# Patryk27/strolle

Hardware: NVIDIA H100
Metric: Mrays/s (+ frames/s) at 1080p-per-GPU Cornell, ReSTIR DI+GI + SVGF; H100 vs CPU restatement of the reference (higher is better)
Workload: dtype f32

## Files before the change

include/strolle_b200.h:

```cpp
#ifndef STROLLE_B200_H
#define STROLLE_B200_H

#include <stddef.h>
#include <stdint.h>

#ifdef __cplusplus
extern "C" {
#endif

typedef struct st_engine st_engine;
typedef uint64_t st_handle;
typedef int32_t st_camera_handle;

enum { ST_OK = 0, ST_ERR_CUDA = -1, ST_ERR_INVALID = -2, ST_ERR_NOT_FOUND = -3, ST_ERR_LIMIT = -4 };

typedef struct st_mesh_triangle {
    float positions[3][3];
    float normals[3][3];
    float uvs[3][2];
    float tangents[3][4];
} st_mesh_triangle;

typedef struct st_material {
    float base_color[4];
// ... 46 lines not shown
typedef struct st_material_textures { st_handle base_color, emissive, metallic_roughness, normal_map; uint32_t mask; } st_material_textures;
int st_set_material_textures(st_engine* e, st_handle material, const st_material_textures* textures);
int st_insert_instance(st_engine* e, st_handle instance, st_handle mesh, st_handle material, const float affine[12]);
int st_remove_instance(st_engine* e, st_handle instance);
int st_insert_light(st_engine* e, st_handle light, const st_light* l);
int st_remove_light(st_engine* e, st_handle light);
int st_update_sun(st_engine* e, float azimuth, float altitude);

int st_create_camera(st_engine* e, const st_camera* camera, st_camera_handle* out);
int st_update_camera(st_engine* e, st_camera_handle camera, const st_camera* desc);
int st_delete_camera(st_engine* e, st_camera_handle camera);

int st_tick(st_engine* e);

int st_render_camera(st_engine* e, st_camera_handle camera, void* host_out, int format);
int st_copy_output(st_engine* e, st_camera_handle camera, void* host_out, int format);
int st_synchronize(st_engine* e);

int st_set_seed_base(st_engine* e, uint32_t base);
int st_set_blue_noise(st_engine* e, const uint8_t* rgba8_256x256);
int st_read_buffer(st_engine* e, st_camera_handle camera, const char* name, float* dst, size_t cap_floats, size_t* count);
int st_read_scene(st_engine* e, const char* name, float* dst, size_t cap_floats, size_t* count);
int st_bvh_depth(st_engine* e, int* depth);
uint32_t st_frame(st_engine* e);
int st_set_frame(st_engine* e, uint32_t frame);
int st_trace_closest(st_engine* e, const float* rays, size_t n, float* out, float* device_ms);
int st_trace_any(st_engine* e, const float* rays, size_t n, uint32_t* out, float* device_ms);
int st_device_math(st_engine* e, int op, const float* a, const float* b, float* out, size_t n);
#define ST_PASS_COUNT 27
int st_enable_timing(st_engine* e, int enabled);
int st_pass_times(st_engine* e, float* ms, uint32_t* launches, int reset);
const char* st_pass_name(int pass);
int st_wavelet_times(st_engine* e, float* ms5, uint32_t* launches5, int reset);
enum { ST_OPT_SVGF_FAST_MATH = 1, ST_OPT_ASYNC_OUTPUT = 2, ST_OPT_HALO_NCCL = 3, ST_OPT_WAVELET_TILED = 4, ST_OPT_WAVELET_TILE_CFG = 5, ST_OPT_FUSE_REPROJECT = 6, ST_OPT_BVH_REUSE = 7, ST_OPT_VARIANCE_TILED = 8, ST_OPT_SHADING_FAST_MATH = 9, ST_OPT_STRIP_FUSED = 10, ST_OPT_FUSED_PASSES = 11, ST_OPT_STRIP_DMA = 12, ST_OPT_WAVELET_PAIRED = 13 };
#define ST_WAVELET_PAIRED_DEFAULT 1
#define ST_STRIP_DMA_DEFAULT (-1)
#define ST_FUSED_PASSES_DEFAULT 1
#define ST_SHADING_FAST_DEFAULT 1
#define ST_VARIANCE_TILED_DEFAULT 1
#define ST_WAVELET_TILED_DEFAULT 15
#define ST_WAVELET_CFG_DEFAULT 0x01000
#define ST_FUSE_REPROJECT_DEFAULT 1
int st_set_option(st_engine* e, int option, int value);
enum { ST_STAT_WAVELET_TILED_LAUNCHES = 1, ST_STAT_WAVELET_TILED_ERRORS = 2, ST_STAT_BVH_GRAFTED_SUBTREES = 3, ST_STAT_VARIANCE_TILED_LAUNCHES = 4,
       ST_STAT_STRIP_PULLED_ROWS = 5 , ST_STAT_LAST_FRAME_FUSED_STRIPS = 6 ,
       ST_STAT_STRIP_FIRST_TIMEOUT = 7  };
int st_get_stat(st_engine* e, int stat, uint64_t* value);
typedef struct st_bvh_builder st_bvh_builder;
int st_bvh_builder_create(st_bvh_builder** out);
void st_bvh_builder_destroy(st_bvh_builder* b);
int st_bvh_builder_build(st_bvh_builder* b, const float* prims11, size_t n, int reuse, float* out, size_t cap_floats, size_t* n_floats,
                         uint32_t* grafted_subtrees, int* depth);
int st_bvh_builder_read(st_bvh_builder* b, float* out, size_t cap_floats);
int st_set_stream(st_engine* e, void* cuda_stream, int external);
int st_count_rays(st_engine* e, int enabled);
int st_ray_count(st_engine* e, uint64_t* rays, int reset);
int st_nccl_unique_id(uint8_t* out128);
int st_nccl_init(st_engine* e, const uint8_t* id128, int rank, int world);
int st_plan_frame(const int* schedule, int n, uint32_t frame, int temporal_reach, char* out, size_t cap);
int st_render_strips(st_engine* e, st_camera_handle camera, void* host_out, int format, int temporal_reach, int gather);
int st_plan_strip_order(const int* schedule, int n, int dma, char* out, size_t cap);
int st_strip_bounds(int height, int world, int* rows_out);
int st_halo_bytes(st_engine* e, uint64_t* bytes);
#define ST_PEER_HANDLE_BYTES 192
int st_peer_export(st_engine* e, st_camera_handle camera, uint8_t* out192);
int st_peer_import(st_engine* e, st_camera_handle camera, const uint8_t* all_handles, int rank, int world);
int st_peer_errors(st_engine* e, st_camera_handle camera, uint32_t* count);
// ... 45 lines not shown
```

rust/strolle-b200-sys/src/lib.rs:

```rust
#![allow(non_camel_case_types, clippy::too_many_arguments)]

use std::os::raw::{c_char, c_int, c_void};

#[repr(C)] pub struct st_engine { _private: [u8; 0] }
#[repr(C)] pub struct st_multi { _private: [u8; 0] }
#[repr(C)] pub struct st_bvh_builder { _private: [u8; 0] }
pub type st_handle = u64;
pub type st_camera_handle = i32;

pub const ST_OK: c_int = 0;
pub const ST_ERR_CUDA: c_int = -1;
pub const ST_ERR_INVALID: c_int = -2;
pub const ST_ERR_NOT_FOUND: c_int = -3;
pub const ST_ERR_LIMIT: c_int = -4;

#[repr(C)] #[derive(Clone, Copy, Debug, Default)]
pub struct st_mesh_triangle { pub positions: [[f32; 3]; 3], pub normals: [[f32; 3]; 3], pub uvs: [[f32; 2]; 3], pub tangents: [[f32; 4]; 3] }
#[repr(C)] #[derive(Clone, Copy, Debug, Default)]
pub struct st_material { pub base_color: [f32; 4], pub emissive: [f32; 4], pub perceptual_roughness: f32, pub metallic: f32, pub reflectance: f32, pub ior: f32, pub alpha_blend: i32 }
#[repr(C)] #[derive(Clone, Copy, Debug, Default)]
pub struct st_material_textures { pub base_color: st_handle, pub emissive: st_handle, pub metallic_roughness: st_handle, pub normal_map: st_handle, pub mask: u32 }
pub const ST_LIGHT_POINT: i32 = 1;
pub const ST_LIGHT_SPOT: i32 = 2;
#[repr(C)] #[derive(Clone, Copy, Debug, Default)]
pub struct st_light { pub kind: i32, pub position: [f32; 3], pub radius: f32, pub color: [f32; 3], pub range: f32, pub direction: [f32; 3], pub angle: f32 }
pub const ST_MODE_IMAGE: i32 = 0;
pub const ST_MODE_DI_DIFFUSE: i32 = 1;
pub const ST_MODE_DI_SPECULAR: i32 = 2;
pub const ST_MODE_GI_DIFFUSE: i32 = 3;
pub const ST_MODE_GI_SPECULAR: i32 = 4;
pub const ST_MODE_BVH_HEATMAP: i32 = 5;
pub const ST_MODE_REFERENCE: i32 = 6;
#[repr(C)] #[derive(Clone, Copy, Debug)]
pub struct st_camera { pub mode: i32, pub denoise: i32, pub ref_depth: i32, pub width: u32, pub height: u32, pub transform: [f32; 16], pub projection: [f32; 16] }
pub const ST_FORMAT_RGBA32F: c_int = 0;
pub const ST_FORMAT_RGBA8_SRGB: c_int = 1;
pub const ST_PASS_COUNT: usize = 27;
pub const ST_PEER_HANDLE_BYTES: usize = 192;

pub const ST_OPT_SVGF_FAST_MATH: c_int = 1;
pub const ST_OPT_ASYNC_OUTPUT: c_int = 2;
pub const ST_OPT_HALO_NCCL: c_int = 3;
pub const ST_OPT_WAVELET_TILED: c_int = 4;
pub const ST_OPT_WAVELET_TILE_CFG: c_int = 5;
pub const ST_OPT_FUSE_REPROJECT: c_int = 6;
pub const ST_OPT_BVH_REUSE: c_int = 7;
pub const ST_OPT_VARIANCE_TILED: c_int = 8;
pub const ST_OPT_SHADING_FAST_MATH: c_int = 9;
pub const ST_OPT_STRIP_FUSED: c_int = 10;
pub const ST_OPT_FUSED_PASSES: c_int = 11;
pub const ST_OPT_STRIP_DMA: c_int = 12;
pub const ST_OPT_WAVELET_PAIRED: c_int = 13;
pub const ST_STAT_WAVELET_TILED_LAUNCHES: c_int = 1;
pub const ST_STAT_WAVELET_TILED_ERRORS: c_int = 2;
pub const ST_STAT_BVH_GRAFTED_SUBTREES: c_int = 3;
pub const ST_STAT_VARIANCE_TILED_LAUNCHES: c_int = 4;
pub const ST_STAT_STRIP_PULLED_ROWS: c_int = 5;
pub const ST_STAT_LAST_FRAME_FUSED_STRIPS: c_int = 6;
pub const ST_STAT_STRIP_FIRST_TIMEOUT: c_int = 7;
pub const ST_WAVELET_PAIRED_DEFAULT: c_int = 1;
pub const ST_STRIP_DMA_DEFAULT: c_int = -1;
pub const ST_FUSED_PASSES_DEFAULT: c_int = 1;
pub const ST_SHADING_FAST_DEFAULT: c_int = 1;
pub const ST_VARIANCE_TILED_DEFAULT: c_int = 1;
pub const ST_WAVELET_TILED_DEFAULT: c_int = 15;
pub const ST_WAVELET_CFG_DEFAULT: c_int = 0x01000;
pub const ST_FUSE_REPROJECT_DEFAULT: c_int = 1;

#[link(name = "strolle_b200")]
extern "C" {
    pub fn st_last_error() -> *const c_char;
    pub fn st_engine_create(device: c_int, out: *mut *mut st_engine) -> c_int;
    pub fn st_engine_destroy(e: *mut st_engine);
    pub fn st_insert_mesh(e: *mut st_engine, mesh: st_handle, triangles: *const st_mesh_triangle, count: usize) -> c_int;
    pub fn st_remove_mesh(e: *mut st_engine, mesh: st_handle) -> c_int;
    pub fn st_insert_material(e: *mut st_engine, material: st_handle, m: *const st_material) -> c_int;
    pub fn st_has_material(e: *mut st_engine, material: st_handle) -> c_int;
    pub fn st_remove_material(e: *mut st_engine, material: st_handle) -> c_int;
    pub fn st_insert_image(e: *mut st_engine, image: st_handle, rgba8: *const u8, width: u32, height: u32) -> c_int;
    pub fn st_remove_image(e: *mut st_engine, image: st_handle) -> c_int;
    pub fn st_set_material_textures(e: *mut st_engine, material: st_handle, textures: *const st_material_textures) -> c_int;
    pub fn st_insert_instance(e: *mut st_engine, instance: st_handle, mesh: st_handle, material: st_handle, affine: *const f32) -> c_int;
    pub fn st_remove_instance(e: *mut st_engine, instance: st_handle) -> c_int;
    pub fn st_insert_light(e: *mut st_engine, light: st_handle, l: *const st_light) -> c_int;
    pub fn st_remove_light(e: *mut st_engine, light: st_handle) -> c_int;
    pub fn st_update_sun(e: *mut st_engine, azimuth: f32, altitude: f32) -> c_int;
    pub fn st_create_camera(e: *mut st_engine, camera: *const st_camera, out: *mut st_camera_handle) -> c_int;
    pub fn st_update_camera(e: *mut st_engine, camera: st_camera_handle, desc: *const st_camera) -> c_int;
    pub fn st_delete_camera(e: *mut st_engine, camera: st_camera_handle) -> c_int;
    pub fn st_tick(e: *mut st_engine) -> c_int;
    pub fn st_render_camera(e: *mut st_engine, camera: st_camera_handle, host_out: *mut c_void, format: c_int) -> c_int;
    pub fn st_copy_output(e: *mut st_engine, camera: st_camera_handle, host_out: *mut c_void, format: c_int) -> c_int;
// ... 72 lines not shown
```

strolle_b200/csrc/engine.cu:

```cuda
#include <algorithm>
#include <cmath>
#include <cstdio>
#include <cstring>
#include <deque>
#include <functional>
#include <limits>
#include <string>
#include <unordered_map>
#include <vector>

#include <nccl.h>

#include "../../include/strolle_b200.h"
#include "kernels.h"

#include <dlfcn.h>
namespace {
struct NcclApi {
    void* lib = nullptr;
    ncclResult_t (*GetUniqueId)(ncclUniqueId*) = nullptr;
    ncclResult_t (*CommInitRank)(ncclComm_t*, int, ncclUniqueId, int) = nullptr;
    ncclResult_t (*CommDestroy)(ncclComm_t) = nullptr;
    ncclResult_t (*GroupStart)() = nullptr;
    ncclResult_t (*GroupEnd)() = nullptr;
// ... 300 lines not shown
    }
    void release() { if (p) cudaFree(p); p = nullptr; cap = 0; }
};

static const char* kPassNames[P_COUNT] = {
    "prim_gbuffer", "di_sampling", "di_temporal_resampling", "di_spatial_resampling_pick", "di_spatial_resampling_trace", "di_spatial_resampling_sample",
    "di_resolving", "gi_reprojection", "gi_sampling_a", "gi_sampling_b", "gi_temporal_resampling", "gi_spatial_resampling_pick",
    "gi_spatial_resampling_trace", "gi_spatial_resampling_sample", "gi_preview_resampling", "gi_resolving", "frame_reprojection",
    "frame_denoising_reproject", "frame_denoising_estimate_variance", "frame_denoising_wavelet", "frame_composition", "ref_tracing",
    "ref_shading", "bvh_heatmap", "atmosphere", "trace_stream", "halo_exchange"};

static uint32_t dispatch_seed(uint32_t base, uint32_t frame, uint32_t k) {
    uint32_t s = base ^ (frame * 64u + k);
    s = s * 747796405u + 2891336453u;
    uint32_t w = ((s >> ((s >> 28) + 4u)) ^ s) * 277803737u;
    return (w >> 22) ^ w;
}

struct CameraSlot {
    bool alive = false;
    st_camera desc;
    uint32_t frame = 0;
    CameraDev dev;
    std::vector<std::pair<std::string, float4**>> named;
    std::vector<std::pair<std::string, size_t>> sizes;
    DevMem arena;
    DevMem svgf_pairs; float4* pair[2] = {nullptr, nullptr};
    DevMem rgba8; int rgba8_slot = 0;
    cudaEvent_t ev_ready[2] = {nullptr, nullptr}, ev_copied[2] = {nullptr, nullptr};
    cudaStream_t side[2] = {nullptr, nullptr}; cudaEvent_t ev_produced = nullptr, ev_pushed[2] = {nullptr, nullptr}; bool pushed_pending[2] = {false, false};
    struct PeerLink { bool ready = false; bool ipc = false; std::vector<char*> arena, rgba8; std::vector<uint32_t*> flags; DevMem sync; uint32_t seq = 0, fseq = 0; } peer;
};

struct Step { int pass; std::function<void(cudaStream_t)> run; int sub = -1; };

}

using namespace st;

struct st_engine {
    int device = 0;
    cudaStream_t stream = nullptr; bool own_stream = true;
    cudaStream_t copy_stream = nullptr;
    std::unordered_map<st_handle, std::vector<st_mesh_triangle>> meshes;
    std::vector<st_material> materials; std::vector<st_handle> material_handles; bool materials_dirty = false;
    struct MatTex { st_handle tex[4]; uint32_t mask; };
    std::vector<MatTex> material_textures;
    struct ImageRect { st_handle handle; uint32_t x, y, w, h; };
    std::vector<ImageRect> images; uint32_t shelf_x = 0, shelf_y = 0, shelf_h = 0; bool images_dirty = false;
    DevMem d_atlas, d_srgb, d_tri_instance, d_instance_xforms;
    bool motion_dirty = true;
    bool moved_last_tick = false;
    struct Inst { st_handle handle, mesh, material; Affine3 xf, xf_inv, prev_xf; bool dirty; };
    std::vector<Inst> instances; bool instances_dirty = false;
    struct Range { st_handle handle; size_t b, e; };
    std::vector<Range> tri_ranges; SlotAllocator tri_alloc;
    std::vector<float4> h_triangles; std::vector<Prim> prims; bool triangles_dirty = false;
    BvhBuild bvh; BvhOut bvh_out; bool bvh_dirty = false;
    std::vector<GpuMaterial> h_materials;
    static const st_handle kSun = ~(st_handle)0;
    std::vector<GpuLight> h_lights; std::vector<std::pair<st_handle, uint32_t>> light_slots;
    std::vector<st_handle> lights_created, lights_updated; std::vector<std::pair<st_handle, uint32_t>> lights_remapped; std::vector<uint32_t> lights_killed;
    uint32_t next_light = 1; bool lights_dirty = true;
    float sun_azimuth = 0.0f, sun_altitude = 0.35f; bool sun_dirty = true;
    GpuWorld world;
    uint32_t frame = 1, seed_base = 0xC0FFEEu;
    DevMem d_triangles, d_bvh, d_materials, d_matpacked, d_unpacklut, d_lights, d_noise, d_tlut, d_slut, d_skylut, d_scratch, d_raycount;
    bool count_rays = false;
    bool svgf_fast = true;
    bool shading_fast = ST_SHADING_FAST_DEFAULT != 0;
    bool fused_passes = ST_FUSED_PASSES_DEFAULT != 0;
    bool async_output = false;
    bool halo_nccl = false;
    int wavelet_paired = ST_WAVELET_PAIRED_DEFAULT;
    int strip_dma = ST_STRIP_DMA_DEFAULT;
    bool strip_fused = true;
    bool last_frame_fused = false;
    int wavelet_tiled = ST_WAVELET_TILED_DEFAULT;
    int wavelet_cfg = ST_WAVELET_CFG_DEFAULT;
    DevMem d_tile_errors; uint64_t wavelet_tiled_launches = 0;
    bool fuse_reproject = ST_FUSE_REPROJECT_DEFAULT != 0;
    bool bvh_reuse = true;
    bool variance_tiled = ST_VARIANCE_TILED_DEFAULT != 0; uint64_t variance_tiled_launches = 0;
    bool luts_static_ready = false, sky_ready = false; float sky_for_altitude = 0.0f;
    std::vector<CameraSlot*> cameras;
    bool timing = false;
    float pass_ms[P_COUNT] = {}; uint32_t pass_launches[P_COUNT] = {};
    float wavelet_ms[5] = {}; uint32_t wavelet_launches[5] = {};
    struct Timed { int pass; cudaEvent_t a, b; int sub; };
    std::vector<Timed> pending; std::vector<cudaEvent_t> event_pool;
    cudaEvent_t mark_a = nullptr, mark_b = nullptr;
    ncclComm_t comm = nullptr; int rank = 0, n_ranks = 1;
    uint64_t halo_bytes_last_frame = 0;

    SceneDev scene() const {
        SceneDev s;
        s.triangles = (const float4*)d_triangles.p; s.bvh = (const float4*)d_bvh.p; s.bvh_len = (uint32_t)bvh_out.buf.size(); s.materials = (const GpuMaterial*)d_materials.p;
        s.lights = (const GpuLight*)d_lights.p; s.blue_noise = (const uchar4*)d_noise.p;
        s.transmittance_lut = (const float4*)d_tlut.p; s.scattering_lut = (const float4*)d_slut.p; s.sky_lut = (const float4*)d_skylut.p;
        s.world = world;
        s.tri_instance = (const uint32_t*)d_tri_instance.p; s.instance_xforms = (const float4*)d_instance_xforms.p;
        s.atlas = (const uchar4*)d_atlas.p; s.srgb_lut = (const float*)d_srgb.p;
        s.material_packed = (const uint32_t*)d_matpacked.p; s.unpack_lut = (const float*)d_unpacklut.p;
        s.ray_counter = count_rays ? (unsigned long long*)d_raycount.p : nullptr;
        return s;
    }
    uint32_t* light_slot(st_handle h) { for (auto& p : light_slots) if (p.first == h) return &p.second; return nullptr; }
    cudaEvent_t get_event() { if (!event_pool.empty()) { cudaEvent_t e = event_pool.back(); event_pool.pop_back(); return e; } cudaEvent_t e; cudaEventCreate(&e); return e; }
    void run_timed(int pass, const std::function<void(cudaStream_t)>& fn, int sub = -1) {
        if (!timing) { fn(stream); pass_launches[pass]++; return; }
        Timed t; t.pass = pass; t.sub = sub; t.a = get_event(); t.b = get_event();
        cudaEventRecord(t.a, stream); fn(stream); cudaEventRecord(t.b, stream);
        pending.push_back(t); pass_launches[pass]++;
    }
    void collect_timing() {
        for (Timed& t : pending) { cudaEventSynchronize(t.b); float ms = 0; cudaEventElapsedTime(&ms, t.a, t.b); pass_ms[t.pass] += ms; if (t.pass == P_DENOISE_WAVELET && t.sub >= 0 && t.sub < 5) { wavelet_ms[t.sub] += ms; wavelet_launches[t.sub]++; } event_pool.push_back(t.a); event_pool.push_back(t.b); }
// ... 166 lines not shown
    const CameraDev camG = grown(cam, x.gbuffer), camV = grown(cam, x.variance);
    const int pm0 = x.preview_mirror[0], pm1 = x.preview_mirror[1];
    const SceneDev sc = e->scene();
    const uint32_t f = cs->frame;
    const int cur = (f % 2u) == 1u ? 1 : 0;
    const st_camera& d = cs->desc;
    const bool fs = e->shading_fast;
    auto seed = [&](uint32_t k) { return dispatch_seed(e->seed_base, f, k); };
    auto add = [&](int pass, std::function<void(cudaStream_t)> fn) { steps->push_back(Step{pass, std::move(fn)}); };
    const float4* di_final = (d.denoise && (d.mode == ST_MODE_IMAGE || d.mode == ST_MODE_DI_DIFFUSE)) ? cam.di_diff_curr_colors : cam.di_diff_samples;
    const float4* gi_final = (d.denoise && (d.mode == ST_MODE_IMAGE || d.mode == ST_MODE_GI_DIFFUSE)) ? cam.gi_diff_curr_colors : cam.gi_diff_samples;
    if (d.mode == ST_MODE_BVH_HEATMAP) {
        add(P_BVH_HEATMAP, [=](cudaStream_t s) { launch_bvh_heatmap(cam, sc, s); });
        add(P_COMPOSITION, [=](cudaStream_t s) { launch_composition(cam, sc, cur, 5u, di_final, gi_final, s); });
        return;
    }
    if (d.mode == ST_MODE_REFERENCE) {
        for (uint32_t depth = 0; depth <= (uint32_t)d.ref_depth; depth++) {
            uint32_t sd = seed(P_REF_SHADING_SEED + depth);
            add(P_REF_TRACING, [=](cudaStream_t s) { launch_ref_tracing(cam, sc, depth, s); });
            add(P_REF_SHADING, [=](cudaStream_t s) { launch_ref_shading(cam, sc, sd, depth, s); });
        }
        add(P_REF_SHADING, [=](cudaStream_t s) { launch_ref_shading(cam, sc, 0u, 255u, s); });
        add(P_COMPOSITION, [=](cudaStream_t s) { launch_composition(cam, sc, cur, 6u, di_final, gi_final, s); });
        return;
    }
    const bool needs_di = d.mode == ST_MODE_IMAGE || d.mode == ST_MODE_DI_DIFFUSE || d.mode == ST_MODE_DI_SPECULAR;
    const bool needs_gi = d.mode == ST_MODE_IMAGE || d.mode == ST_MODE_GI_DIFFUSE || d.mode == ST_MODE_GI_SPECULAR;
    const int k4_in_k0 = (e->fused_passes && (ext == nullptr || ext->still) && !e->instances.empty()) ? 1 : 0;
    add(P_PRIM_GBUFFER, [=](cudaStream_t s) { launch_prim_gbuffer(camG, sc, cur, k4_in_k0, s); });
    const bool fp = e->fused_passes;
    if (!e->instances.empty()) {
        if (!k4_in_k0) add(P_FRAME_REPROJECTION, [=](cudaStream_t s) { launch_frame_reprojection(cam, sc, cur, s); });
        if (needs_di) {
            uint32_t s1 = seed(P_DI_SAMPLING), s2 = seed(P_DI_TEMPORAL), s3 = seed(P_DI_SPATIAL_PICK), s5 = seed(P_DI_SPATIAL_SAMPLE);
            if (fp) {
                add(P_DI_TEMPORAL, [=](cudaStream_t s) { (fs ? stf::launch_di_sample_temporal : st::launch_di_sample_temporal)(cam, sc, cur, s1, s2, f, s); });
                add(P_DI_SPATIAL_PICK, [=](cudaStream_t s) { (fs ? stf::launch_di_spatial_fused : st::launch_di_spatial_fused)(cam, sc, cur, s3, s5, f, s); });
            } else {
                add(P_DI_SAMPLING, [=](cudaStream_t s) { (fs ? stf::launch_di_sampling : st::launch_di_sampling)(cam, sc, cur, s1, f, s); });
                add(P_DI_TEMPORAL, [=](cudaStream_t s) { (fs ? stf::launch_di_temporal : st::launch_di_temporal)(cam, sc, cur, s2, s); });
                add(P_DI_SPATIAL_PICK, [=](cudaStream_t s) { (fs ? stf::launch_di_spatial_pick : st::launch_di_spatial_pick)(cam, sc, cur, s3, f, s); });
                add(P_DI_SPATIAL_TRACE, [=](cudaStream_t s) { (fs ? stf::launch_spatial_trace : st::launch_spatial_trace)(cam, sc, cam.di_diff_samples, cam.di_diff_curr_colors, cam.di_diff_stash, s); });
                add(P_DI_SPATIAL_SAMPLE, [=](cudaStream_t s) { (fs ? stf::launch_di_spatial_sample : st::launch_di_spatial_sample)(cam, sc, s5, f, s); });
            }
            add(P_DI_RESOLVING, [=](cudaStream_t s) { (fs ? stf::launch_di_resolving : st::launch_di_resolving)(cam, sc, cur, s); });
        }
        if (needs_gi) {
            uint32_t sa = seed(P_GI_SAMPLING_A), sb = seed(P_GI_SAMPLING_B), st_ = seed(P_GI_TEMPORAL), sp = seed(P_GI_SPATIAL_PICK), ss = seed(P_GI_SPATIAL_SAMPLE), sv = seed(P_GI_PREVIEW);
            uint32_t source;
            const bool tracing = f % 6u < 4u;
            const int inline_rp = (fp && tracing) ? 1 : 0;
            if (!inline_rp) add(P_GI_REPROJECTION, [=](cudaStream_t s) { (fs ? stf::launch_gi_reprojection : st::launch_gi_reprojection)(cam, sc, cur, s); });
            auto sampling = [&]() {
                if (fp) { add(P_GI_SAMPLING_B, [=](cudaStream_t s) { (fs ? stf::launch_gi_sampling_fused : st::launch_gi_sampling_fused)(cam, sc, cur, sa, sb, f, s); }); return; }
                add(P_GI_SAMPLING_A, [=](cudaStream_t s) { (fs ? stf::launch_gi_sampling_a : st::launch_gi_sampling_a)(cam, sc, cur, sa, f, s); });
                add(P_GI_SAMPLING_B, [=](cudaStream_t s) { (fs ? stf::launch_gi_sampling_b : st::launch_gi_sampling_b)(cam, sc, cur, sb, f, s); });
            };
            if (tracing) {
                if (f % 2u == 0u) sampling();
                add(P_GI_TEMPORAL, [=](cudaStream_t s) { (fs ? stf::launch_gi_temporal : st::launch_gi_temporal)(cam, sc, cur, st_, f, inline_rp, s); });
                if (f % 2u == 1u) {
                    if (fp) add(P_GI_SPATIAL_PICK, [=](cudaStream_t s) { (fs ? stf::launch_gi_spatial_fused : st::launch_gi_spatial_fused)(cam, sc, cur, sp, ss, f, s); });
                    else {
                        add(P_GI_SPATIAL_PICK, [=](cudaStream_t s) { (fs ? stf::launch_gi_spatial_pick : st::launch_gi_spatial_pick)(cam, sc, cur, sp, f, s); });
                        add(P_GI_SPATIAL_TRACE, [=](cudaStream_t s) { (fs ? stf::launch_spatial_trace : st::launch_spatial_trace)(cam, sc, cam.gi_d0, cam.gi_d1, cam.gi_d2, s); });
                        add(P_GI_SPATIAL_SAMPLE, [=](cudaStream_t s) { (fs ? stf::launch_gi_spatial_sample : st::launch_gi_spatial_sample)(cam, sc, ss, f, s); });
                    }
                    source = 1;
                } else source = 0;
            } else {
                sampling();
                add(P_GI_TEMPORAL, [=](cudaStream_t s) { (fs ? stf::launch_gi_temporal : st::launch_gi_temporal)(cam, sc, cur, st_, f, 0, s); });
                source = 0;
            }
            const float4* src0 = source == 0 ? cam.gi_reservoirs[1] : cam.gi_reservoirs[2];
            add(P_GI_PREVIEW, [=](cudaStream_t s) { (fs ? stf::launch_gi_preview : st::launch_gi_preview)(cam, sc, cur, sv, 0u, src0, cam.gi_reservoirs[3], pm0, s); });
            if (fp) add(P_GI_PREVIEW, [=](cudaStream_t s) { (fs ? stf::launch_gi_preview_resolve : st::launch_gi_preview_resolve)(cam, sc, cur, sv, cam.gi_reservoirs[3], src0, s); });
            else {
                add(P_GI_PREVIEW, [=](cudaStream_t s) { (fs ? stf::launch_gi_preview : st::launch_gi_preview)(cam, sc, cur, sv, 1u, cam.gi_reservoirs[3], cam.gi_reservoirs[0], pm1, s); });
                add(P_GI_RESOLVING, [=](cudaStream_t s) { (fs ? stf::launch_gi_resolving : st::launch_gi_resolving)(cam, sc, cur, src0, s); });
            }
        }
    }
    if (d.denoise) {
        if (e->fuse_reproject) {
            add(P_DENOISE_REPROJECT, [=](cudaStream_t s) { launch_denoise_reproject_pair(cam, sc, cur, s); });
        } else {
            add(P_DENOISE_REPROJECT, [=](cudaStream_t s) { launch_denoise_reproject(cam, sc, cur, cam.di_diff_prev_colors, cam.di_diff_moments[cur ^ 1], cam.di_diff_samples, cam.di_diff_curr_colors, cam.di_diff_moments[cur], s); });
            add(P_DENOISE_REPROJECT, [=](cudaStream_t s) { launch_denoise_reproject(cam, sc, cur, cam.gi_diff_prev_colors, cam.gi_diff_moments[cur ^ 1], cam.gi_diff_samples, cam.gi_diff_curr_colors, cam.gi_diff_moments[cur], s); });
        }
        const bool fast = e->svgf_fast;
        const bool var_tiled = e->variance_tiled; uint32_t* verr = (uint32_t*)e->d_tile_errors.p;
        add(P_DENOISE_VARIANCE, [=](cudaStream_t s) {
            if (var_tiled && launch_denoise_variance_tiled(camV, sc, cur, fast, verr, s)) { e->variance_tiled_launches++; return; }
            launch_denoise_variance(camV, sc, cur, fast, s);
        });
        float4* di_io[5][2] = {{cam.di_diff_stash, cam.di_diff_prev_colors}, {cam.di_diff_prev_colors, cam.di_diff_stash}, {cam.di_diff_stash, cam.di_diff_curr_colors},
                               {cam.di_diff_curr_colors, cam.di_diff_stash}, {cam.di_diff_stash, cam.di_diff_curr_colors}};
        float4* gi_io[5][2] = {{cam.gi_diff_stash, cam.gi_diff_prev_colors}, {cam.gi_diff_prev_colors, cam.gi_diff_stash}, {cam.gi_diff_stash, cam.gi_diff_curr_colors},
                               {cam.gi_diff_curr_colors, cam.gi_diff_stash}, {cam.gi_diff_stash, cam.gi_diff_curr_colors}};
        const bool whole_or_fused = ext != nullptr || (cam.y0 == 0 && cam.y1 == cam.h);
        const int first_paired_read = (fast && whole_or_fused && cs->pair[0]) ? (e->wavelet_paired == 2 ? 3 : e->wavelet_paired == 1 ? 4 : 5) : 5;
        for (uint32_t nth = 0; nth < 5; nth++) {
            float4 *a = di_io[nth][0], *b = di_io[nth][1], *c = gi_io[nth][0], *g = gi_io[nth][1];
            const bool reads_pair = (int)nth >= first_paired_read, writes_pair = (int)nth + 1 >= first_paired_read && nth < 4;
            const float4* pin = reads_pair ? cs->pair[nth & 1] : nullptr; float4* pout = writes_pair ? cs->pair[(nth + 1) & 1] : nullptr;
            const bool tiled = !reads_pair && ((e->wavelet_tiled >> nth) & 1) != 0; const int cfg = (e->wavelet_cfg >> (4 * nth)) & 15;
            uint32_t* terr = (uint32_t*)e->d_tile_errors.p;
            const CameraDev camW = grown(cam, x.wavelet[nth]);
            add(P_DENOISE_WAVELET, [=](cudaStream_t s) {
                if (tiled && launch_denoise_wavelet_tiled(camW, sc, f, 1u << nth, (float)(1 + nth), a, b, c, g, pout, fast, cfg, terr, s)) { e->wavelet_tiled_launches++; return; }
                launch_denoise_wavelet(camW, sc, cur, f, 1u << nth, (float)(1 + nth), a, b, c, g, pin, pout, fast, s);
            });
            steps->back().sub = (int)nth;
        }
    }
    uint32_t mode = (uint32_t)d.mode;
    add(P_COMPOSITION, [=](cudaStream_t s) { launch_composition(cam, sc, cur, mode, di_final, gi_final, s); });
}


struct HaloItem { std::string name; int reach; };
struct HaloExchange { int before_step; std::vector<HaloItem> items; };
static const int kSpatialReach = 128;
static const int kPreview2Reach = 64;
static const int kVarianceReach = 3;
static const int kWaveletReach[5] = {1, 2, 4, 9, 19};

static void plan_frame(const int* schedule, int n, uint32_t frame, int temporal_reach, std::vector<HaloExchange>* plan) {
    const char* cur = (frame % 2u == 1u) ? "b" : "a";
    const char* prv = (frame % 2u == 1u) ? "a" : "b";
    bool have_gbuffer = false; int nth_preview = 0, nth_wavelet = 0;
    const char* wavelet_inputs[5] = {"stash", "prev_colors", "stash", "curr_colors", "stash"};
    bool has_preview = false, has_gi_spatial = false;
    for (int i = 0; i < n; i++) { if (schedule[i] == P_GI_PREVIEW) has_preview = true; if (schedule[i] == P_GI_SPATIAL_PICK) has_gi_spatial = true; }
    std::string gi_source = has_gi_spatial ? "gi_reservoirs_2" : "gi_reservoirs_1";
    for (int i = 0; i < n; i++) {
        int p = schedule[i];
        HaloExchange ex; ex.before_step = i;
        auto add = [&](const std::string& name, int reach) { ex.items.push_back({name, reach}); };
        if (i == 0 && temporal_reach > 0) {
            add(std::string("prim_surface_map_") + prv, temporal_reach); add(std::string("prim_gbuffer_d0_") + prv, temporal_reach); add(std::string("prim_gbuffer_d1_") + prv, temporal_reach);
            add("di_reservoirs_0", temporal_reach); add("gi_reservoirs_0", temporal_reach); add("di_diff_prev_colors", temporal_reach); add("gi_diff_prev_colors", temporal_reach);
            add(std::string("di_diff_moments_") + prv, temporal_reach); add(std::string("gi_diff_moments_") + prv, temporal_reach);
        }
        if (p == P_DI_SPATIAL_PICK || p == P_GI_SPATIAL_PICK) {
            if (!have_gbuffer) { add(std::string("prim_gbuffer_d0_") + cur, kSpatialReach); add(std::string("prim_gbuffer_d1_") + cur, kSpatialReach); add("surface_nd", kSpatialReach); have_gbuffer = true; }
            add(p == P_DI_SPATIAL_PICK ? "di_reservoirs_1" : "gi_reservoirs_1", kSpatialReach);
        } else if (p == P_GI_PREVIEW) {
            if (nth_preview == 0) {
                add(std::string("prim_surface_map_") + cur, kSpatialReach); add(gi_source, kSpatialReach);
// ... 273 lines not shown
    if (!out) return fail(ST_ERR_INVALID, "out is null");
    int count = 0;
    cudaError_t ce = cudaGetDeviceCount(&count);
    if (ce != cudaSuccess || count == 0) return fail(ST_ERR_CUDA, "no CUDA device available: this library has no CPU fallback");
    if (device < 0 || device >= count) return fail(ST_ERR_INVALID, "bad device ordinal");
    CK(cudaSetDevice(device));
    st_engine* e = new st_engine();
    e->device = device;
    CK(cudaStreamCreateWithFlags(&e->stream, cudaStreamNonBlocking));
    std::memset(&e->world, 0, sizeof e->world);
    e->h_lights.push_back(make_sun(make_float4(0, 0, 0, 25.0f), make_float4(0, 0, 0, std::numeric_limits<float>::infinity())));
    e->light_slots.push_back({st_engine::kSun, 0u});
    int rc = e->d_noise.ensure(256 * 256 * 4); if (rc) { delete e; return rc; }
    rc = e->d_unpacklut.ensure(512 * 4); if (rc) { delete e; return rc; }
    rc = e->d_tile_errors.ensure(4); if (rc) { delete e; return rc; }
    launch_unpack_lut((float*)e->d_unpacklut.p, e->stream);
    *out = e;
    return ST_OK;
}
void st_engine_destroy(st_engine* e) {
    if (!e) return;
    cudaSetDevice(e->device);
    cudaStreamSynchronize(e->stream);
    if (e->copy_stream) cudaStreamSynchronize(e->copy_stream);
    for (CameraSlot* c : e->cameras) { for (int k = 0; k < 2; k++) { if (c->side[k]) { cudaStreamSynchronize(c->side[k]); cudaStreamDestroy(c->side[k]); } if (c->ev_pushed[k]) cudaEventDestroy(c->ev_pushed[k]); } if (c->ev_produced) cudaEventDestroy(c->ev_produced);
        c->arena.release(); c->svgf_pairs.release(); c->rgba8.release(); for (int k = 0; k < 2; k++) { if (c->ev_ready[k]) cudaEventDestroy(c->ev_ready[k]); if (c->ev_copied[k]) cudaEventDestroy(c->ev_copied[k]); } delete c; }
    DevMem* all[] = {&e->d_triangles, &e->d_bvh, &e->d_materials, &e->d_lights, &e->d_noise, &e->d_tlut, &e->d_slut, &e->d_skylut, &e->d_scratch, &e->d_raycount, &e->d_matpacked, &e->d_unpacklut, &e->d_atlas, &e->d_srgb, &e->d_tri_instance, &e->d_instance_xforms, &e->d_tile_errors};
    for (DevMem* d : all) d->release();
    for (auto& t : e->pending) { cudaEventDestroy(t.a); cudaEventDestroy(t.b); }
    for (cudaEvent_t ev : e->event_pool) cudaEventDestroy(ev);
    if (e->comm) g_nccl.CommDestroy(e->comm);
    if (e->own_stream) cudaStreamDestroy(e->stream);
    if (e->copy_stream) cudaStreamDestroy(e->copy_stream);
    delete e;
}

int st_insert_mesh(st_engine* e, st_handle mesh, const st_mesh_triangle* tris, size_t count) {
    if (!e || (!tris && count)) return fail(ST_ERR_INVALID, "null argument");
    e->meshes[mesh].assign(tris, tris + count);
    return ST_OK;
}
int st_remove_mesh(st_engine* e, st_handle mesh) { if (!e) return fail(ST_ERR_INVALID, "null engine"); e->meshes.erase(mesh); return ST_OK; }

int st_insert_material(st_engine* e, st_handle h, const st_material* m) {
    if (!e || !m) return fail(ST_ERR_INVALID, "null argument");
    auto it = std::find(e->material_handles.begin(), e->material_handles.end(), h);
    if (it != e->material_handles.end()) e->materials[it - e->material_handles.begin()] = *m;
    else { e->material_handles.push_back(h); e->materials.push_back(*m); st_engine::MatTex mt; std::memset(&mt, 0, sizeof mt); e->material_textures.push_back(mt); }
    e->materials_dirty = true;
    return ST_OK;
}
int st_has_material(st_engine* e, st_handle h) { return e && std::find(e->material_handles.begin(), e->material_handles.end(), h) != e->material_handles.end() ? 1 : 0; }
int st_remove_material(st_engine* e, st_handle h) {
    if (!e) return fail(ST_ERR_INVALID, "null engine");
    auto it = std::find(e->material_handles.begin(), e->material_handles.end(), h);
    if (it != e->material_handles.end()) *it = ~(st_handle)0 - 1;
    e->materials_dirty = true;
    return ST_OK;
}

int st_insert_image(st_engine* e, st_handle h, const uint8_t* rgba8, uint32_t w, uint32_t hgt) {
    if (!e || !rgba8 || w == 0 || hgt == 0) return fail(ST_ERR_INVALID, "null argument");
    CK(cudaSetDevice(e->device));
    int rc;
    if (!e->d_atlas.p) {
        if ((rc = e->d_atlas.ensure((size_t)kAtlasSize * kAtlasSize * 4))) return rc;
// ... 209 lines not shown
        for (auto& r : e->lights_remapped) e->h_lights[r.second].d3.x = bits2f(*e->light_slot(r.first) + 1u);
        if ((rc = upload(e, e->d_lights, e->h_lights.data(), e->h_lights.size() * sizeof(GpuLight)))) return rc;
        CK(cudaStreamSynchronize(e->stream));
        bool again = !e->lights_created.empty() || !e->lights_updated.empty() || !e->lights_killed.empty() || !e->lights_remapped.empty();
        for (st_handle h : e->lights_created) { GpuLight& l = e->h_lights[*e->light_slot(h)]; l.prev_d0 = l.d0; l.prev_d1 = l.d1; l.prev_d2 = l.d2; }
        for (st_handle h : e->lights_updated) { GpuLight& l = e->h_lights[*e->light_slot(h)]; l.prev_d0 = l.d0; l.prev_d1 = l.d1; l.prev_d2 = l.d2; }
        for (uint32_t id : e->lights_killed) e->h_lights[id].d3.x = 0.0f;
        for (auto& r : e->lights_remapped) e->h_lights[r.second].d3.x = 0.0f;
        e->lights_created.clear(); e->lights_updated.clear(); e->lights_remapped.clear(); e->lights_killed.clear();
        e->lights_dirty = again;
    }
    for (CameraSlot* c : e->cameras) if (c->alive) c->frame = e->frame;
    e->frame += 1;
    if (too_deep) return fail(ST_ERR_LIMIT, "BVH deeper than the 24-entry traversal stack (strolle-gpu/src/lib.rs:72-76): the scene is not drawn until it changes");
    return ST_OK;
}

int st_frame_schedule(st_engine* e, st_camera_handle h, int* pass_ids, int cap, int* count) {
    CameraSlot* cs = e ? get_camera(e, h) : nullptr;
    if (!cs || !count) return fail(ST_ERR_NOT_FOUND, "unknown camera");
    std::vector<Step> steps; build_schedule(e, cs, &steps);
    *count = (int)steps.size();
    for (int i = 0; i < cap && i < *count; i++) pass_ids[i] = steps[i].pass;
    return ST_OK;
}
int st_render_range(st_engine* e, st_camera_handle h, int first, int last) {
    CameraSlot* cs = e ? get_camera(e, h) : nullptr;
    if (!cs) return fail(ST_ERR_NOT_FOUND, "unknown camera");
    if (cs->frame == 0) return fail(ST_ERR_INVALID, "st_tick must precede st_render_camera");
    CK(cudaSetDevice(e->device));
    int rc = ensure_luts(e); if (rc) return rc;
    std::vector<Step> steps; build_schedule(e, cs, &steps);
    if (last < 0 || last >= (int)steps.size()) last = (int)steps.size() - 1;
    for (int i = std::max(first, 0); i <= last; i++) e->run_timed(steps[i].pass, steps[i].run, steps[i].sub);
    CK(cudaGetLastError());
    return ST_OK;
}
int st_render_camera(st_engine* e, st_camera_handle h, void* host_out, int format) {
    int rc = st_render_range(e, h, 0, -1); if (rc) return rc;
    if (host_out) return st_copy_output(e, h, host_out, format);
    return ST_OK;
}
static int copy_rows_out(st_engine* e, CameraSlot* cs, void* host_out, int format, int y0, int y1) {
    const size_t W = cs->desc.width, n = W * cs->desc.height;
    const size_t first = (size_t)y0 * W, count = (size_t)(y1 - y0) * W;
    if (format == ST_FORMAT_RGBA32F) CK(cudaMemcpyAsync((char*)host_out + first * 16, cs->dev.output + first, count * 16, cudaMemcpyDeviceToHost, e->stream));
    else if (format == ST_FORMAT_RGBA8_SRGB) {
        int rc2 = cs->rgba8.ensure(2 * n * 4); if (rc2) return rc2;
        cs->rgba8_slot ^= 1;
        SceneDev sc = e->scene(); uchar4* dst8 = (uchar4*)cs->rgba8.p + (cs->rgba8_slot ? n : 0); CameraDev cd = cs->dev; cd.y0 = y0; cd.y1 = y1;
        const int k = cs->rgba8_slot;
        if (e->async_output) {
            if (!e->copy_stream) CK(cudaStreamCreateWithFlags(&e->copy_stream, cudaStreamNonBlocking));
            if (!cs->ev_ready[k]) { CK(cudaEventCreateWithFlags(&cs->ev_ready[k], cudaEventDisableTiming)); CK(cudaEventCreateWithFlags(&cs->ev_copied[k], cudaEventDisableTiming)); }
            else CK(cudaStreamWaitEvent(e->stream, cs->ev_copied[k], 0));
        }
        e->run_timed(P_COMPOSITION, [=](cudaStream_t s) { launch_output_rgba8(cd, sc, dst8, s); });
        if (e->async_output) {
            CK(cudaEventRecord(cs->ev_ready[k], e->stream));
            CK(cudaStreamWaitEvent(e->copy_stream, cs->ev_ready[k], 0));
            CK(cudaMemcpyAsync((char*)host_out + first * 4, dst8 + first, count * 4, cudaMemcpyDeviceToHost, e->copy_stream));
            CK(cudaEventRecord(cs->ev_copied[k], e->copy_stream));
        } else CK(cudaMemcpyAsync((char*)host_out + first * 4, dst8 + first, count * 4, cudaMemcpyDeviceToHost, e->stream));
    } else return fail(ST_ERR_INVALID, "unsupported output format");
    return ST_OK;
}
int st_copy_output(st_engine* e, st_camera_handle h, void* host_out, int format) {
// ... 79 lines not shown
}
int st_trace_closest(st_engine* e, const float* rays, size_t n, float* out, float* ms) { return trace_stream(e, rays, n, out, true, ms); }
int st_trace_any(st_engine* e, const float* rays, size_t n, uint32_t* out, float* ms) { return trace_stream(e, rays, n, out, false, ms); }

int st_device_math(st_engine* e, int op, const float* a, const float* b, float* out, size_t n) {
    if (!e || !a || !out) return fail(ST_ERR_INVALID, "null argument");
    CK(cudaSetDevice(e->device));
    DevMem da, db, dc; int rc;
    if ((rc = da.ensure(n * 4)) || (rc = db.ensure(n * 4)) || (rc = dc.ensure(n * 4))) return rc;
    CK(cudaMemcpyAsync(da.p, a, n * 4, cudaMemcpyHostToDevice, e->stream));
    if (b) CK(cudaMemcpyAsync(db.p, b, n * 4, cudaMemcpyHostToDevice, e->stream));
    launch_math(op, (const float*)da.p, (const float*)db.p, (float*)dc.p, (long)n, e->stream);
    CK(cudaMemcpyAsync(out, dc.p, n * 4, cudaMemcpyDeviceToHost, e->stream));
    CK(cudaStreamSynchronize(e->stream));
    da.release(); db.release(); dc.release();
    return ST_OK;
}

int st_set_option(st_engine* e, int option, int value) {
    if (!e) return fail(ST_ERR_INVALID, "null engine");
    if (option == ST_OPT_SVGF_FAST_MATH) { e->svgf_fast = value != 0; return ST_OK; }
    if (option == ST_OPT_SHADING_FAST_MATH) { e->shading_fast = value != 0; return ST_OK; }
    if (option == ST_OPT_ASYNC_OUTPUT) { e->async_output = value != 0; return ST_OK; }
    if (option == ST_OPT_HALO_NCCL) { e->halo_nccl = value != 0; return ST_OK; }
    if (option == ST_OPT_STRIP_FUSED) { e->strip_fused = value != 0; return ST_OK; }
    if (option == ST_OPT_STRIP_DMA) { if (value < -1 || value > 3) return fail(ST_ERR_INVALID, "ST_OPT_STRIP_DMA: -1 .. 3"); e->strip_dma = value; return ST_OK; }
    if (option == ST_OPT_WAVELET_PAIRED) { if (value < 0 || value > 2) return fail(ST_ERR_INVALID, "ST_OPT_WAVELET_PAIRED: 0, 1 or 2"); e->wavelet_paired = value; return ST_OK; }
    if (option == ST_OPT_FUSED_PASSES) { e->fused_passes = value != 0; return ST_OK; }
    if (option == ST_OPT_WAVELET_TILED) { e->wavelet_tiled = value & 31; return ST_OK; }
    if (option == ST_OPT_VARIANCE_TILED) { e->variance_tiled = value != 0; return ST_OK; }
    if (option == ST_OPT_BVH_REUSE) { e->bvh_reuse = value != 0; return ST_OK; }
    if (option == ST_OPT_FUSE_REPROJECT) { e->fuse_reproject = value != 0; return ST_OK; }
    if (option == ST_OPT_WAVELET_TILE_CFG) { e->wavelet_cfg = value & 0xfffff; return ST_OK; }
    return fail(ST_ERR_INVALID, "unknown option");
}
struct st_bvh_builder { BvhBuild b; BvhOut flat; };
int st_bvh_builder_create(st_bvh_builder** out) { if (!out) return fail(ST_ERR_INVALID, "out is null"); *out = new st_bvh_builder(); return ST_OK; }
void st_bvh_builder_destroy(st_bvh_builder* b) { delete b; }
int st_bvh_builder_read(st_bvh_builder* b, float* out, size_t cap_floats) {
    if (!b || !out) return fail(ST_ERR_INVALID, "null argument");
    if (cap_floats < b->flat.buf.size() * 4) return fail(ST_ERR_LIMIT, "output buffer too small");
    std::memcpy(out, b->flat.buf.data(), b->flat.buf.size() * 16);
    return ST_OK;
}
int st_bvh_builder_build(st_bvh_builder* b, const float* prims11, size_t n, int reuse, float* out, size_t cap_floats, size_t* n_floats, uint32_t* grafted, int* depth) {
    if (!b || (!prims11 && n) || !n_floats) return fail(ST_ERR_INVALID, "null argument");
    std::vector<Prim> all(n);
    uint32_t max_mat = 0;
    for (size_t i = 0; i < n; i++) {
        const float* f = prims11 + 11 * i;
        Prim& p = all[i];
        p.tri = f2bits(f[0]); p.mat = f2bits(f[1]); p.center = h3(f[2], f[3], f[4]);
        p.box.lo = h3(f[5], f[6], f[7]); p.box.hi = h3(f[8], f[9], f[10]);
        max_mat = std::max(max_mat, p.mat);
    }
    b->b.build(all, reuse != 0);
    for (const Prim& p : b->b.prims) max_mat = std::max(max_mat, p.mat);
    std::vector<uint8_t> alpha((size_t)max_mat + 1, 0);
    b->b.flatten(alpha, &b->flat);
    *n_floats = b->flat.buf.size() * 4;
    if (grafted) *grafted = b->b.grafted;
    if (depth) *depth = b->flat.depth;
    if (out) return st_bvh_builder_read(b, out, cap_floats);
    return ST_OK;
}

// ... 440 lines not shown
```

strolle_b200/engine.py:

```python
import ctypes as C
import os

import numpy as np

_HERE = os.path.dirname(os.path.abspath(__file__))
PASS_COUNT = 27
FORMAT_RGBA32F, FORMAT_RGBA8_SRGB = 0, 1
OPT_SVGF_FAST_MATH = 1
OPT_ASYNC_OUTPUT = 2
OPT_HALO_NCCL = 3
OPT_WAVELET_TILED = 4
OPT_WAVELET_TILE_CFG = 5
OPT_FUSE_REPROJECT = 6
OPT_BVH_REUSE = 7
OPT_VARIANCE_TILED = 8
OPT_FUSED_PASSES = 11
OPT_WAVELET_PAIRED = 13
OPT_STRIP_DMA = 12
OPT_STRIP_FUSED = 10
OPT_SHADING_FAST_MATH = 9
WAVELET_TILED_DEFAULT = 15
STAT_WAVELET_TILED_LAUNCHES = 1
STAT_WAVELET_TILED_ERRORS = 2
STAT_BVH_GRAFTED_SUBTREES = 3
STAT_VARIANCE_TILED_LAUNCHES = 4
STAT_STRIP_PULLED_ROWS = 5
STAT_LAST_FRAME_FUSED_STRIPS = 6
STAT_STRIP_FIRST_TIMEOUT = 7


class StrolleError(RuntimeError):
    pass


def lib_path():
    return os.environ.get("STROLLE_B200_LIB") or os.path.join(_HERE, "_lib", "libstrolle_b200.so")


class _MeshTriangle(C.Structure):
    _fields_ = [("positions", C.c_float * 9), ("normals", C.c_float * 9), ("uvs", C.c_float * 6), ("tangents", C.c_float * 12)]


class _Material(C.Structure):
    _fields_ = [("base_color", C.c_float * 4), ("emissive", C.c_float * 4), ("perceptual_roughness", C.c_float), ("metallic", C.c_float),
                ("reflectance", C.c_float), ("ior", C.c_float), ("alpha_blend", C.c_int32)]


class _MaterialTextures(C.Structure):
    _fields_ = [("base_color", C.c_uint64), ("emissive", C.c_uint64), ("metallic_roughness", C.c_uint64), ("normal_map", C.c_uint64), ("mask", C.c_uint32)]


class _Light(C.Structure):
    _fields_ = [("kind", C.c_int32), ("position", C.c_float * 3), ("radius", C.c_float), ("color", C.c_float * 3), ("range", C.c_float),
# ... 541 lines not shown
```

Before: 3692.

## Run ReSTIR DI and GI pass chains concurrently on a second stream

Marks the GI pass chain to run on a separate non-blocking stream, forked from the main stream with an event at the start of the DI chain and joined back before denoising. The DI and GI kernels can then overlap on the GPU and fill SMs that either chain alone leaves idle. It adds event record/wait overhead and the risk of hidden data dependencies between the DI and GI passes. It is only enabled for single-rank image mode with denoising and timing off.

Result: faster. 3784 (median of 6 runs) (+2.5%).

```diff
diff --git a/include/strolle_b200.h b/include/strolle_b200.h
--- a/include/strolle_b200.h
+++ b/include/strolle_b200.h
@@ -102,7 +102,8 @@
 int st_pass_times(st_engine* e, float* ms, uint32_t* launches, int reset);
 const char* st_pass_name(int pass);
 int st_wavelet_times(st_engine* e, float* ms5, uint32_t* launches5, int reset);
-enum { ST_OPT_SVGF_FAST_MATH = 1, ST_OPT_ASYNC_OUTPUT = 2, ST_OPT_HALO_NCCL = 3, ST_OPT_WAVELET_TILED = 4, ST_OPT_WAVELET_TILE_CFG = 5, ST_OPT_FUSE_REPROJECT = 6, ST_OPT_BVH_REUSE = 7, ST_OPT_VARIANCE_TILED = 8, ST_OPT_SHADING_FAST_MATH = 9, ST_OPT_STRIP_FUSED = 10, ST_OPT_FUSED_PASSES = 11, ST_OPT_STRIP_DMA = 12, ST_OPT_WAVELET_PAIRED = 13 };
+enum { ST_OPT_SVGF_FAST_MATH = 1, ST_OPT_ASYNC_OUTPUT = 2, ST_OPT_HALO_NCCL = 3, ST_OPT_WAVELET_TILED = 4, ST_OPT_WAVELET_TILE_CFG = 5, ST_OPT_FUSE_REPROJECT = 6, ST_OPT_BVH_REUSE = 7, ST_OPT_VARIANCE_TILED = 8, ST_OPT_SHADING_FAST_MATH = 9, ST_OPT_STRIP_FUSED = 10, ST_OPT_FUSED_PASSES = 11, ST_OPT_STRIP_DMA = 12, ST_OPT_WAVELET_PAIRED = 13, ST_OPT_CONCURRENT_CHAINS = 14 };
+#define ST_CONCURRENT_CHAINS_DEFAULT 1
 #define ST_WAVELET_PAIRED_DEFAULT 1
 #define ST_STRIP_DMA_DEFAULT (-1)
 #define ST_FUSED_PASSES_DEFAULT 1
diff --git a/rust/strolle-b200-sys/src/lib.rs b/rust/strolle-b200-sys/src/lib.rs
--- a/rust/strolle-b200-sys/src/lib.rs
+++ b/rust/strolle-b200-sys/src/lib.rs
@@ -51,6 +51,7 @@
 pub const ST_OPT_FUSED_PASSES: c_int = 11;
 pub const ST_OPT_STRIP_DMA: c_int = 12;
 pub const ST_OPT_WAVELET_PAIRED: c_int = 13;
+pub const ST_OPT_CONCURRENT_CHAINS: c_int = 14;
 pub const ST_STAT_WAVELET_TILED_LAUNCHES: c_int = 1;
 pub const ST_STAT_WAVELET_TILED_ERRORS: c_int = 2;
 pub const ST_STAT_BVH_GRAFTED_SUBTREES: c_int = 3;
@@ -58,6 +59,7 @@
 pub const ST_STAT_STRIP_PULLED_ROWS: c_int = 5;
 pub const ST_STAT_LAST_FRAME_FUSED_STRIPS: c_int = 6;
 pub const ST_STAT_STRIP_FIRST_TIMEOUT: c_int = 7;
+pub const ST_CONCURRENT_CHAINS_DEFAULT: c_int = 1;
 pub const ST_WAVELET_PAIRED_DEFAULT: c_int = 1;
 pub const ST_STRIP_DMA_DEFAULT: c_int = -1;
 pub const ST_FUSED_PASSES_DEFAULT: c_int = 1;
diff --git a/strolle_b200/csrc/engine.cu b/strolle_b200/csrc/engine.cu
--- a/strolle_b200/csrc/engine.cu
+++ b/strolle_b200/csrc/engine.cu
@@ -356,7 +356,7 @@
     struct PeerLink { bool ready = false; bool ipc = false; std::vector<char*> arena, rgba8; std::vector<uint32_t*> flags; DevMem sync; uint32_t seq = 0, fseq = 0; } peer;
 };
 
-struct Step { int pass; std::function<void(cudaStream_t)> run; int sub = -1; };
+struct Step { int pass; std::function<void(cudaStream_t)> run; int sub = -1; int lane = 0; bool fork = false; };
 
 }
 
@@ -366,6 +366,7 @@
     int device = 0;
     cudaStream_t stream = nullptr; bool own_stream = true;
     cudaStream_t copy_stream = nullptr;
+    cudaStream_t chain_stream = nullptr;
     std::unordered_map<st_handle, std::vector<st_mesh_triangle>> meshes;
     std::vector<st_material> materials; std::vector<st_handle> material_handles; bool materials_dirty = false;
     struct MatTex { st_handle tex[4]; uint32_t mask; };
@@ -406,6 +407,7 @@
     bool fuse_reproject = ST_FUSE_REPROJECT_DEFAULT != 0;
     bool bvh_reuse = true;
     bool variance_tiled = ST_VARIANCE_TILED_DEFAULT != 0; uint64_t variance_tiled_launches = 0;
+    bool concurrent_chains = ST_CONCURRENT_CHAINS_DEFAULT != 0;
     bool luts_static_ready = false, sky_ready = false; float sky_for_altitude = 0.0f;
     std::vector<CameraSlot*> cameras;
     bool timing = false;
@@ -638,6 +640,7 @@
     const bool fp = e->fused_passes;
     if (!e->instances.empty()) {
         if (!k4_in_k0) add(P_FRAME_REPROJECTION, [=](cudaStream_t s) { launch_frame_reprojection(cam, sc, cur, s); });
+        const size_t di_first = steps->size();
         if (needs_di) {
             uint32_t s1 = seed(P_DI_SAMPLING), s2 = seed(P_DI_TEMPORAL), s3 = seed(P_DI_SPATIAL_PICK), s5 = seed(P_DI_SPATIAL_SAMPLE);
             if (fp) {
@@ -652,6 +655,7 @@
             }
             add(P_DI_RESOLVING, [=](cudaStream_t s) { (fs ? stf::launch_di_resolving : st::launch_di_resolving)(cam, sc, cur, s); });
         }
+        const size_t gi_first = steps->size();
         if (needs_gi) {
             uint32_t sa = seed(P_GI_SAMPLING_A), sb = seed(P_GI_SAMPLING_B), st_ = seed(P_GI_TEMPORAL), sp = seed(P_GI_SPATIAL_PICK), ss = seed(P_GI_SPATIAL_SAMPLE), sv = seed(P_GI_PREVIEW);
             uint32_t source;
@@ -688,6 +692,11 @@
                 add(P_GI_RESOLVING, [=](cudaStream_t s) { (fs ? stf::launch_gi_resolving : st::launch_gi_resolving)(cam, sc, cur, src0, s); });
             }
         }
+        const bool lanes = e->concurrent_chains && !e->timing && ext == nullptr && e->n_ranks == 1 && d.mode == ST_MODE_IMAGE && d.denoise;
+        if (lanes && di_first < gi_first && gi_first < steps->size()) {
+            (*steps)[di_first].fork = true;
+            for (size_t i = gi_first; i < steps->size(); i++) (*steps)[i].lane = 1;
+        }
     }
     if (d.denoise) {
         if (e->fuse_reproject) {
@@ -724,6 +733,31 @@
     }
     uint32_t mode = (uint32_t)d.mode;
     add(P_COMPOSITION, [=](cudaStream_t s) { launch_composition(cam, sc, cur, mode, di_final, gi_final, s); });
+}
+
+static int run_steps(st_engine* e, const std::vector<Step>& steps, int first, int last) {
+    auto order = [e](cudaStream_t before, cudaStream_t after) {
+        cudaEvent_t ev = e->get_event();
+        cudaError_t ce = cudaEventRecord(ev, before);
+        if (ce == cudaSuccess) ce = cudaStreamWaitEvent(after, ev, 0);
+        e->event_pool.push_back(ev);
+        return ce == cudaSuccess ? ST_OK : fail(ST_ERR_CUDA, std::string("chain fork / join: ") + cudaGetErrorString(ce));
+    };
+    bool forked = false, open = false;
+    int rc;
+    for (int i = first; i <= last; i++) {
+        const Step& s = steps[i];
+        if (!forked && (s.fork || s.lane == 1)) {
+            if (!e->chain_stream) CK(cudaStreamCreateWithFlags(&e->chain_stream, cudaStreamNonBlocking));
+            if ((rc = order(e->stream, e->chain_stream))) return rc;
+            forked = true;
+        }
+        if (s.lane == 1) { s.run(e->chain_stream); e->pass_launches[s.pass]++; open = true; continue; }
+        if (open) { if ((rc = order(e->chain_stream, e->stream))) return rc; open = false; }
+        e->run_timed(s.pass, s.run, s.sub);
+    }
+    if (open && (rc = order(e->chain_stream, e->stream))) return rc;
+    return ST_OK;
 }
 
 
@@ -1063,6 +1097,7 @@
     if (e->comm) g_nccl.CommDestroy(e->comm);
     if (e->own_stream) cudaStreamDestroy(e->stream);
     if (e->copy_stream) cudaStreamDestroy(e->copy_stream);
+    if (e->chain_stream) cudaStreamDestroy(e->chain_stream);
     delete e;
 }
 
@@ -1338,7 +1373,7 @@
     int rc = ensure_luts(e); if (rc) return rc;
     std::vector<Step> steps; build_schedule(e, cs, &steps);
     if (last < 0 || last >= (int)steps.size()) last = (int)steps.size() - 1;
-    for (int i = std::max(first, 0); i <= last; i++) e->run_timed(steps[i].pass, steps[i].run, steps[i].sub);
+    if ((rc = run_steps(e, steps, std::max(first, 0), last))) return rc;
     CK(cudaGetLastError());
     return ST_OK;
 }
@@ -1484,6 +1519,7 @@
     if (option == ST_OPT_BVH_REUSE) { e->bvh_reuse = value != 0; return ST_OK; }
     if (option == ST_OPT_FUSE_REPROJECT) { e->fuse_reproject = value != 0; return ST_OK; }
     if (option == ST_OPT_WAVELET_TILE_CFG) { e->wavelet_cfg = value & 0xfffff; return ST_OK; }
+    if (option == ST_OPT_CONCURRENT_CHAINS) { e->concurrent_chains = value != 0; return ST_OK; }
     return fail(ST_ERR_INVALID, "unknown option");
 }
 struct st_bvh_builder { BvhBuild b; BvhOut flat; };
diff --git a/strolle_b200/engine.py b/strolle_b200/engine.py
--- a/strolle_b200/engine.py
+++ b/strolle_b200/engine.py
@@ -19,6 +19,7 @@
 OPT_STRIP_DMA = 12
 OPT_STRIP_FUSED = 10
 OPT_SHADING_FAST_MATH = 9
+OPT_CONCURRENT_CHAINS = 14
 WAVELET_TILED_DEFAULT = 15
 STAT_WAVELET_TILED_LAUNCHES = 1
 STAT_WAVELET_TILED_ERRORS = 2
```
